# maltezfaria/LevelSetMethods.jl

Measured on AMD Instinct MI355X. Metric: Mcells/s per RK3 step (WENO5 advect+reinit), 512^3 fp64; HBM GB/s vs peak, higher is better.
Workload: dtype f64; 1 GPU; 3D 512^3 vortex-deformation WENO5 advection + EikonalReinitializationTerm, RK3, NeumannBC, fp64; cells=134217728, integrator=RK3, arithmetic_mode=fast, parallelism=single, halo_overlap=n/a, prewarm_steps=10, exchange=n/a

## Files before the change

### levelsetmethods.jl_amd/csrc/stage_kernel.h

```cpp
#pragma once
#include <cstdlib>
#include <type_traits>
#include "lsm_internal.h"
#include "stage_math.h"

namespace lsm {
namespace LSM_NS {

#if LSM_STRICT
#define LSM_LDS7 0
#define LSM_ZD 0
constexpr bool ADV_SCALED = false;
#else
constexpr bool ADV_SCALED = true;
#endif
constexpr int adv_factor_kind(int ADV, bool PLAIN) {
#if LSM_STRICT
    return 0;
#else
    return ADV == 2 ? (LSM_T1 ? 1 : 0) | (LSM_T2 && PLAIN ? 2 : 0) : 0;
#endif
}
template <int FK>
LSM_DEV double adv_factor(const StageArgs& a, int k) {
    if constexpr (FK == 3) return a.cdt_inv_h3[k];
    else if constexpr (FK == 2) return a.cdt * a.inv_h[k];
    else if constexpr (FK == 1) return a.inv_h3[k];
    else return a.inv_h[k];
}

constexpr int halo_of(int ADV, int NM, int CURV, int EIK) {
    int g = 0;
    if (ADV == 2) g = 3;
    if (ADV == 1 && g < 1) g = 1;
    if ((NM || EIK) && g < 2) g = 2;
    if (CURV && g < 1) g = 1;
    return g;
}

template <class T>
LSM_DEV T* uniform_ptr(T* p) {
    const unsigned long long v = reinterpret_cast<unsigned long long>(p);
    const unsigned lo = __builtin_amdgcn_readfirstlane((unsigned)v), hi = __builtin_amdgcn_readfirstlane((unsigned)(v >> 32));
    return reinterpret_cast<T*>(((unsigned long long)hi << 32) | lo);
}
LSM_DEV double ld_uniform(const double* t, int i) {
    typedef const __attribute__((address_space(4))) double* cptr;
    return *((cptr)(unsigned long long)t + i);
}
typedef unsigned lsm_v2u __attribute__((ext_vector_type(2)));
LSM_DEV __amdgpu_buffer_rsrc_t plane_rsrc(const void* base, int range = (int)0x80000000u) {
    return __builtin_amdgcn_make_buffer_rsrc(const_cast<void*>(base), 0, range, 0x00020000);
}
constexpr unsigned LSM_OOB_OFFSET = 0xC0000000u;
template <class ST, int AUX = 0>
LSM_DEV double ldg(const ST* base, unsigned boff, int range = (int)0x80000000u) {
    if constexpr (sizeof(ST) == 8) return __builtin_bit_cast(double, __builtin_amdgcn_raw_buffer_load_b64(plane_rsrc(base, range), boff, 0, AUX));
    else return (double)__builtin_bit_cast(float, __builtin_amdgcn_raw_buffer_load_b32(plane_rsrc(base, range), boff, 0, AUX));
}
template <class ST, int AUX = 0>
LSM_DEV void stg(ST* base, unsigned boff, double v) {
    if constexpr (sizeof(ST) == 8) __builtin_amdgcn_raw_buffer_store_b64(__builtin_bit_cast(lsm_v2u, v), plane_rsrc(base), boff, 0, AUX);
    else __builtin_amdgcn_raw_buffer_store_b32(__builtin_bit_cast(unsigned, (float)v), plane_rsrc(base), boff, 0, AUX);
}
typedef unsigned lsm_v4u __attribute__((ext_vector_type(4)));
template <class ST, int AUX = 0>
LSM_DEV void ldg2(const ST* base, unsigned boff, double& x, double& y, int range = (int)0x80000000u) {
    if constexpr (sizeof(ST) == 8) {
        const lsm_v4u v = __builtin_bit_cast(lsm_v4u, __builtin_amdgcn_raw_buffer_load_b128(plane_rsrc(base, range), boff, 0, AUX));
        x = __builtin_bit_cast(double, lsm_v2u{v.x, v.y});
        y = __builtin_bit_cast(double, lsm_v2u{v.z, v.w});
    } else {
        const unsigned long long u = __builtin_bit_cast(unsigned long long, __builtin_amdgcn_raw_buffer_load_b64(plane_rsrc(base, range), boff, 0, AUX));
        x = (double)__builtin_bit_cast(float, (unsigned)u);
        y = (double)__builtin_bit_cast(float, (unsigned)(u >> 32));
    }
}
template <class ST, int AUX = 0>
LSM_DEV void stg2(ST* base, unsigned boff, double x, double y) {
    if constexpr (sizeof(ST) == 8) {
        const lsm_v2u a = __builtin_bit_cast(lsm_v2u, x), b = __builtin_bit_cast(lsm_v2u, y);
        __builtin_amdgcn_raw_buffer_store_b128(lsm_v4u{a.x, a.y, b.x, b.y}, plane_rsrc(base), boff, 0, AUX);
    } else {
        const unsigned long long u = (unsigned long long)__builtin_bit_cast(unsigned, (float)x) | ((unsigned long long)__builtin_bit_cast(unsigned, (float)y) << 32);
        __builtin_amdgcn_raw_buffer_store_b64(__builtin_bit_cast(lsm_v2u, u), plane_rsrc(base), boff, 0, AUX);
    }
}
LSM_DEV unsigned ldg_u8(const unsigned char* base, unsigned boff, int range) {
    return __builtin_amdgcn_raw_buffer_load_b8(
        __builtin_amdgcn_make_buffer_rsrc(const_cast<unsigned char*>(base), 0, __builtin_amdgcn_readfirstlane(range), 0x00020000), boff, 0, 0);
}

template <int NDIM, int NCOMP, bool SCALED = false, int KIND = -1, int FK = 0>
LSM_DEV void coeff_prep(const CoeffArgs& c, const StageArgs& a, int gi0, int gi1, double pre[3]) {
    pre[0] = pre[1] = pre[2] = 0.0;
    const int kind = KIND >= 0 ? KIND : c.kind;
    if (kind == LSM_COEFF_CONST) {
#pragma unroll
        for (int k = 0; k < NCOMP; ++k) pre[k] = SCALED ? c.v[k] * adv_factor<FK>(a, k) : c.v[k];
    } else if (kind == LSM_COEFF_ROTATION) {
        const double x1 = a.lc[0] + (double)gi0 * a.h[0];
        pre[1] = c.v[0] * (x1 - c.v[1]);
        if (SCALED) pre[1] = pre[1] * adv_factor<FK>(a, 1);
        if (NDIM == 3) {
            const double x2 = a.lc[1] + (double)gi1 * a.h[1];
            pre[0] = -(c.v[0] * (x2 - c.v[2]));
            if (SCALED) pre[0] = pre[0] * adv_factor<FK>(a, 0);
        }
    } else if (kind == LSM_COEFF_SEPARABLE) {
#pragma unroll
        for (int k = 0; k < NCOMP; ++k) {
            const double* T = c.sep[k];
            double p = T[gi0];
            if (NDIM == 3) p = p * T[a.gn[0] + gi1];
            pre[k] = SCALED ? p * (c.tfac * adv_factor<FK>(a, k)) : p;
        }
    }
}
template <int NDIM, int NCOMP, bool SCALED = false, int KIND = -1, int FK = 0>
LSM_DEV void coeff_eval(const CoeffArgs& c, const StageArgs& a, const double pre[3], const double tz[3], int gim, long long plane_off,
                        unsigned ocol, double out[3]) {
    const int kind = KIND >= 0 ? KIND : c.kind;
    if (kind == LSM_COEFF_CONST) {
#pragma unroll
        for (int k = 0; k < NCOMP; ++k) out[k] = pre[k];
    } else if (kind == LSM_COEFF_ROTATION) {
        if (NDIM == 2) {
            const double x2 = a.lc[1] + (double)gim * a.h[1];
            out[0] = -(c.v[0] * (x2 - c.v[2]));
            if (SCALED) out[0] = out[0] * adv_factor<FK>(a, 0);
        } else {
            out[0] = pre[0];
        }
        if (NCOMP > 1) out[1] = pre[1];
        if (NCOMP > 2) out[2] = 0.0;
    } else if (kind == LSM_COEFF_SEPARABLE) {
#pragma unroll
        for (int k = 0; k < NCOMP; ++k) {
            double p = pre[k];
            if (NDIM > 1) p = p * tz[k];
            out[k] = SCALED ? p : p * c.tfac;
        }
    } else {
#pragma unroll
        for (int k = 0; k < NCOMP; ++k) {
            out[k] = ldg(uniform_ptr(c.f[k] + plane_off), ocol);
            if (SCALED) out[k] = out[k] * adv_factor<FK>(a, k);
        }
    }
}

struct PlaneTab {
    double adv[3], nm[3], curv[3];
};
template <int NDIM, int NCOMP, int KIND>
LSM_DEV void plane_tab_one(const CoeffArgs& c, const StageArgs& a, int gim, double tz[3]) {
    tz[0] = tz[1] = tz[2] = 1.0;
    if (NDIM > 1 && (KIND >= 0 ? KIND : c.kind) == LSM_COEFF_SEPARABLE) {
#pragma unroll
        for (int k = 0; k < NCOMP; ++k) tz[k] = ld_uniform(c.sep[k], (NDIM == 3 ? a.gn[0] + a.gn[1] : a.gn[0]) + gim);
    }
}
template <int NDIM, int ADV, int NM, int CURV, int AK>
LSM_DEV void plane_tab(const StageArgs& a, int gim, PlaneTab& t) {
    if constexpr (ADV != 0) plane_tab_one<NDIM, NDIM, AK>(a.adv, a, gim, t.adv);
    if constexpr (NM != 0) plane_tab_one<NDIM, 1, (AK >= 0 ? (int)LSM_COEFF_CONST : -1)>(a.nm, a, gim, t.nm);
    if constexpr (CURV != 0) plane_tab_one<NDIM, 1, (AK >= 0 ? (int)LSM_COEFF_CONST : -1)>(a.curv, a, gim, t.curv);
}

struct NodeIO {
    long long plane_off;
    unsigned ocol;
    unsigned ocold;
    int gim;
};

struct NodeOps {
    double u[3];
    double vnm;
    double bcurv;
    double s0;
    double phin;
    double out2;
    bool have_negs;
    unsigned long long negs[3];
};
template <int NDIM, int ADV, int NM, int CURV, int EIK, class ST, int AK>
LSM_DEV void node_operands(const StageArgs& a, const NodeIO& io, const double pre_adv[3], const double pre_nm[3],
                           const double pre_curv[3], const PlaneTab& pt, NodeOps& op) {
    op.u[0] = op.u[1] = op.u[2] = 0.0;
    op.vnm = op.bcurv = op.s0 = op.phin = op.out2 = 0.0;
    op.have_negs = false;
    if constexpr (ADV != 0)
        coeff_eval<NDIM, NDIM, ADV_SCALED, AK, adv_factor_kind(ADV, AK >= 0)>(a.adv, a, pre_adv, pt.adv, io.gim, io.plane_off, io.ocold, op.u);
    if constexpr (NM != 0) {
        double vv[3];
        coeff_eval<NDIM, 1, false, (AK >= 0 ? (int)LSM_COEFF_CONST : -1)>(a.nm, a, pre_nm, pt.nm, io.gim, io.plane_off, io.ocold, vv);
        op.vnm = vv[0];
    }
    if constexpr (CURV != 0) {
        double bb[3];
        coeff_eval<NDIM, 1, false, (AK >= 0 ? (int)LSM_COEFF_CONST : -1)>(a.curv, a, pre_curv, pt.curv, io.gim, io.plane_off, io.ocold, bb);
        op.bcurv = bb[0];
    }
    if constexpr (EIK == 1) op.s0 = ldg(uniform_ptr(a.s0 + io.plane_off), io.ocold);
    op.phin = ldg<ST, 0>(uniform_ptr(reinterpret_cast<const ST*>(a.phin) + io.plane_off), io.ocol,
                  __builtin_amdgcn_readfirstlane(a.base_mode == LSM_BASE_PSI ? 0 : (int)0x80000000u));
    if (AK < 0 && a.out2 && a.out2_accum) op.out2 = ldg(uniform_ptr(reinterpret_cast<const ST*>(a.out2) + io.plane_off), io.ocol);
}

template <int NDIM, int G, int W, int R = 0, int RN = 0, bool ZD_ = false>
struct NodeView {
    static constexpr bool ZD = ZD_;
    const double* T0;
    const double* Tm;
    const double* Tp;
    const double* zl;
    double c;
    LSM_DEV double z(int k) const {
        static_assert(!ZD_, "a ring of differences holds no march-axis values: dz()");
        return zl[RN > 0 ? (R + G + k + RN) % (RN > 0 ? RN : 1) : G + k];
    }
    LSM_DEV double dz(int k) const { return zl[(R + G + k + RN) % (RN > 0 ? RN : 1)]; }
    template <int D>
    LSM_DEV double at(int k) const {
        if constexpr (D == 0) return T0[k];
        else if constexpr (D == 1 && NDIM == 3) return T0[k * W];
        else {
            static_assert(!ZD_ || D < NDIM - 1, "a ring of differences holds no march-axis values");
            return z(k);
        }
    }
    template <int A, int B>
    LSM_DEV double corner(int sa, int sb) const {
        if constexpr (NDIM == 3 && A == 0 && B == 1) return T0[sa + sb * W];
        else {
            const double* P = sb > 0 ? Tp : Tm;
            if constexpr (A == 0) return P[sa];
            else return P[sa * W];
        }
    }
};

#if !LSM_STRICT
LSM_DEV double sel64(int m, double x, double y) {
    return __hiloint2double((__double2hiint(x) & m) | (__double2hiint(y) & ~m), (__double2loint(x) & m) | (__double2loint(y) & ~m));
}
#ifndef LSM_NO_UNIFORM_PATHS
#define LSM_UNIFORM_PATHS 1
#else
#define LSM_UNIFORM_PATHS 0
#endif
template <int NDIM, int D, int G, int W, bool PQ, class NV>
LSM_DEV double weno_term(const NV& nv, const StageArgs& a, double v, bool have_negs, unsigned long long negs_known, double& P, double& Q) {
    const double epsf = 1.0e-99 * a.h2[D];
    auto lds = [&](auto Sc) {
        constexpr int ss = (D == 0 ? 1 : W) * decltype(Sc)::value;
        const double q0 = nv.T0[-3 * ss], q1 = nv.T0[-2 * ss], q2 = nv.T0[-ss], q4 = nv.T0[ss], q5 = nv.T0[2 * ss];
        return weno5_undivided_pq<PQ, LSM_T1 != 0>(q1 - q0, q2 - q1, nv.c - q2, q4 - nv.c, q5 - q4, epsf, P, Q);
    };
    auto reg = [&](auto Sc) {
        constexpr int ss = decltype(Sc)::value;
        if constexpr (NV::ZD) {
            if constexpr (ss > 0)
                return weno5_undivided_pq<PQ, LSM_T1 != 0, true>(nv.dz(-3), nv.dz(-2), nv.dz(-1), nv.dz(0), nv.dz(1), epsf, P, Q,
                                                                 max_abs5(nv.dz(-3), nv.dz(-2), nv.dz(-1), nv.dz(0), nv.dz(1)));
            else
                return weno5_undivided_pq<PQ, LSM_T1 != 0, true>(-nv.dz(2), -nv.dz(1), -nv.dz(0), -nv.dz(-1), -nv.dz(-2), epsf, P, Q,
                                                                 max_abs5(nv.dz(2), nv.dz(1), nv.dz(0), nv.dz(-1), nv.dz(-2)));
        } else {
            return weno5_undivided_pq<PQ, LSM_T1 != 0>(nv.z(-2 * ss) - nv.z(-3 * ss), nv.z(-ss) - nv.z(-2 * ss), nv.c - nv.z(-ss),
                                          nv.z(ss) - nv.c, nv.z(2 * ss) - nv.z(ss), epsf, P, Q);
        }
    };
    constexpr bool IN_LDS = D == 0 || (D == 1 && NDIM == 3);
    double w;
    const unsigned long long negs = have_negs ? negs_known : __builtin_amdgcn_ballot_w64(__double2hiint(v) < 0);
    if (LSM_UNIFORM_PATHS && negs == 0) {
        if constexpr (IN_LDS) w = lds(std::integral_constant<int, 1>{});
        else w = reg(std::integral_constant<int, 1>{});
    } else if (LSM_UNIFORM_PATHS && negs == __builtin_amdgcn_ballot_w64(true)) {
        if constexpr (IN_LDS) w = lds(std::integral_constant<int, -1>{});
        else w = reg(std::integral_constant<int, -1>{});
    } else {
        const int m = ~(__double2hiint(v) >> 31);
        if constexpr (!IN_LDS && NV::ZD) {
            w = weno5_undivided_pq<PQ, LSM_T1 != 0>(sel64(m, nv.dz(-3), -nv.dz(2)), sel64(m, nv.dz(-2), -nv.dz(1)), sel64(m, nv.dz(-1), -nv.dz(0)),
                                                    sel64(m, nv.dz(0), -nv.dz(-1)), sel64(m, nv.dz(1), -nv.dz(-2)), epsf, P, Q);
        } else {
            double q[6];
            if constexpr (IN_LDS) {
                constexpr int st = D == 0 ? 1 : W;
                const int ss = (st & m) | (-st & ~m);
                q[0] = nv.T0[-3 * ss]; q[1] = nv.T0[-2 * ss]; q[2] = nv.T0[-ss];
                q[3] = nv.c;
                q[4] = nv.T0[ss]; q[5] = nv.T0[2 * ss];
            } else {
                q[0] = sel64(m, nv.z(-3), nv.z(3));
                q[1] = sel64(m, nv.z(-2), nv.z(2));
                q[2] = sel64(m, nv.z(-1), nv.z(1));
                q[3] = nv.c;
                q[4] = sel64(m, nv.z(1), nv.z(-1));
                q[5] = sel64(m, nv.z(2), nv.z(-2));
            }
            w = weno5_undivided_pq<PQ, LSM_T1 != 0>(q[1] - q[0], q[2] - q[1], q[3] - q[2], q[4] - q[3], q[5] - q[4], epsf, P, Q);
        }
    }
    return w;
}
#endif

template <int NDIM, int D, int G, int W, class NV>
LSM_DEV double weno_dim(const NV& nv, const StageArgs& a, double v) {
    const bool up = v > 0;
    double q[6];
    if constexpr (D == 0 || (D == 1 && NDIM == 3)) {
        constexpr int st = D == 0 ? 1 : W;
        const int ss = up ? st : -st;
        q[0] = nv.T0[-3 * ss]; q[1] = nv.T0[-2 * ss]; q[2] = nv.T0[-ss];
        q[3] = nv.c;
        q[4] = nv.T0[ss]; q[5] = nv.T0[2 * ss];
    } else {
        q[0] = up ? nv.z(-3) : nv.z(3);
        q[1] = up ? nv.z(-2) : nv.z(2);
        q[2] = up ? nv.z(-1) : nv.z(1);
        q[3] = nv.c;
        q[4] = up ? nv.z(1) : nv.z(-1);
        q[5] = up ? nv.z(2) : nv.z(-2);
    }
    const double hs = up ? a.h[D] : -a.h[D];
    const double ihs = up ? a.inv_h[D] : -a.inv_h[D];
    return weno5_upwind(q, hs, ihs, 1.0e-99 * a.h2[D]);
}

template <int NDIM, int ADV, int NM, int CURV, int EIK, int G, int W, class ST, bool PLAIN, class NV>
LSM_DEV void node_update(const StageArgs& a, const NV& nv, const NodeOps& op, double& r_out, double& r_out2) {
    const double c = nv.c;
    double Ladv = 0.0, Lnm = 0.0, Lcurv = 0.0, Leik = 0.0;
#if LSM_STRICT
    constexpr bool ADV_TO_BASE = false;
#else
    constexpr bool ADV_TO_BASE = (adv_factor_kind(ADV, PLAIN) & 2) != 0;
    constexpr bool EIK_RAW = LSM_T3 && EIK == 2;
#endif
    [[maybe_unused]] double adv_base = 0.0;
    double A[3] = {0, 0, 0}, B[3] = {0, 0, 0};
#if LSM_STRICT
    constexpr bool ENO_FROM_WENO = false;
#else
    constexpr bool ENO_FROM_WENO = ADV == 2 && (NM || EIK);
#endif

    if constexpr (ADV != 0) {
        const double* u = op.u;
        auto one = [&](auto Dc) {
            constexpr int D = decltype(Dc)::value;
            const double v = u[D];
            double der;
            if constexpr (ADV == 2) {
#if LSM_STRICT
                der = weno_dim<NDIM, D, G, W>(nv, a, v);
#else
                const double w = weno_term<NDIM, D, G, W, ENO_FROM_WENO>(nv, a, v, op.have_negs, op.negs[D], A[D], B[D]);
                if constexpr (ADV_TO_BASE) {
                    adv_base = D == 0 ? -(__builtin_fabs(v) * w) : __builtin_fma(-__builtin_fabs(v), w, adv_base);
                    return 0.0;
                } else {
                    return __builtin_fabs(v) * w;
                }
#endif
            } else {
#if LSM_STRICT
                der = v > 0 ? (c - nv.template at<D>(-1)) / a.h[D] : (nv.template at<D>(1) - c) / a.h[D];
#else
                der = v > 0 ? (c - nv.template at<D>(-1)) : (nv.template at<D>(1) - c);
#endif
            }
            return v * der;
        };
        Ladv = one(std::integral_constant<int, 0>{});
        if constexpr (NDIM > 1) Ladv = Ladv + one(std::integral_constant<int, 1>{});
        if constexpr (NDIM > 2) Ladv = Ladv + one(std::integral_constant<int, 2>{});
    }

    if constexpr ((NM || EIK) && !ENO_FROM_WENO) {
        auto pr = [&](auto Dc) {
            constexpr int D = decltype(Dc)::value;
            eno2_pair(nv.template at<D>(-2), nv.template at<D>(-1), c, nv.template at<D>(1), nv.template at<D>(2), a.h[D],
                      a.h2[D], a.inv_h[D], A[D], B[D]);
        };
        pr(std::integral_constant<int, 0>{});
        if constexpr (NDIM > 1) pr(std::integral_constant<int, 1>{});
        if constexpr (NDIM > 2) pr(std::integral_constant<int, 2>{});
    }

    if constexpr (NM) {
        const double v = op.vnm;
#if LSM_STRICT
        double gp = 0.0, gm = 0.0;
#pragma unroll
        for (int d = 0; d < NDIM; ++d) {
            double x = positive(A[d]) * positive(A[d]) + negative(B[d]) * negative(B[d]);
            double y = negative(A[d]) * negative(A[d]) + positive(B[d]) * positive(B[d]);
            if (d == 0) { gp = x; gm = y; } else { gp = gp + x; gm = gm + y; }
        }
        Lnm = positive(v) * lsm_sqrt(gp) + negative(v) * lsm_sqrt(gm);
#else
        double g2 = 0.0;
        const unsigned long long vpos = __builtin_amdgcn_ballot_w64(v > 0);
        if (LSM_UNIFORM_PATHS && vpos == __builtin_amdgcn_ballot_w64(true)) {
            g2 = godunov_sum<NDIM, true>(A, B, a.inv_h2, a.uniform_h != 0);
        } else if (LSM_UNIFORM_PATHS && vpos == 0) {
            g2 = godunov_sum<NDIM, false>(A, B, a.inv_h2, a.uniform_h != 0);
        } else {
            const double sg = v > 0 ? 1.0 : -1.0;
#pragma unroll
            for (int d = 0; d < NDIM; ++d) g2 += godunov_term(sg, A[d], B[d], a.inv_h2[d]);
        }
        Lnm = v * fast_norm(g2);
#endif
    }

    if constexpr (CURV) {
        const double bb[1] = {op.bcurv};
#if LSM_STRICT
        double gr[3] = {0, 0, 0}, Hd[3] = {0, 0, 0};
        double H01 = 0, H02 = 0, H12 = 0;
        auto first = [&](auto Dc) {
            constexpr int D = decltype(Dc)::value;
            const double p1 = nv.template at<D>(1), m1 = nv.template at<D>(-1);
            gr[D] = (p1 - m1) / (2 * a.h[D]);
            Hd[D] = (p1 - 2 * c + m1) / a.h2[D];
        };
        first(std::integral_constant<int, 0>{});
        if constexpr (NDIM > 1) first(std::integral_constant<int, 1>{});
        if constexpr (NDIM > 2) first(std::integral_constant<int, 2>{});
        auto mixed = [&](auto Ac, auto Bc) {
            constexpr int A_ = decltype(Ac)::value, B_ = decltype(Bc)::value;
            const double pp = nv.template corner<A_, B_>(1, 1), pm = nv.template corner<A_, B_>(1, -1);
            const double mp = nv.template corner<A_, B_>(-1, 1), mm = nv.template corner<A_, B_>(-1, -1);
            return ((pp - pm) / (2 * a.h[B_]) - (mp - mm) / (2 * a.h[B_])) / (2 * a.h[A_]);
// ... 184 lines not shown
__device__ __forceinline__ void stage_tile(const StageArgs& a, unsigned tile_id, bool tail_tile, unsigned slot) {
    constexpr bool PLAIN = AK >= 0;
    constexpr bool NOMASK = PLAIN && !MASKED;
    constexpr int CK = PLAIN ? (int)LSM_COEFF_CONST : -1;
    constexpr int G = halo_of(ADV, NM, CURV, EIK);
    constexpr bool HAS_Y = NDIM == 3, MARCH = NDIM >= 2;
    constexpr int LEAD = (CURV && MARCH) ? 1 : 0;
    constexpr bool ZROT = LSM_ZROT && !LSM_STRICT && NDIM == 3 && ADV == 2;
    constexpr int W = TX + 2 * G;
    constexpr int H = HAS_Y ? TY + 2 * G : 1;
    constexpr int HW = H * W;
    constexpr bool LDS7 = LSM_LDS7 && ZROT && LEAD == 0 && PLAIN && !MASKED && !NM && EIK == 2 && (2 * G + 1) * HW * 8 + 64 <= 32768;
    constexpr bool ZD = LSM_ZD && LDS7;
    constexpr int NSLOT = LDS7 ? 2 * G + 1 : (MARCH ? 2 * LEAD + 2 : 1);
    constexpr int NT = TX * TY;
    constexpr int NHX = 2 * G * TY;
    constexpr int WY = CURV ? W : TX;
    constexpr int NHY = HAS_Y ? 2 * G * WY : 0;
    constexpr int NH = NHX + NHY;
    constexpr int HPT = (NH + NT - 1) / NT;
    static_assert(!HAS_Y || TY > 1 || true, "");
    __shared__ double tile[NSLOT * HW];

#ifdef LSM_STAMP
    const unsigned long long st_rb = __builtin_amdgcn_s_memrealtime();
#endif
    if (a.tile_list) tile_id = (unsigned)a.tile_list[tile_id];
    else if (a.tile_active && !a.tile_active[tile_id]) return;
    const unsigned tbx = tile_id % a.nb[0], tby = (tile_id / a.nb[0]) % a.nb[1];
    const unsigned tbm = tile_id / (a.nb[0] * a.nb[1]);

    const int tid = threadIdx.x;
    int tx = tid % TX, ty = tid / TX;
    if constexpr (NDIM == 3 && TX == 32 && TY == 8 && !NOMASK) {
        if (LSM_BAND_PATCH && a.mask) { tx = 8 * (tid >> 6) + (tid & 7); ty = (tid & 63) >> 3; }
    }
    const int bx0 = tbx * TX, by0 = HAS_Y ? tby * TY : 0;
    const int gx = bx0 + tx, gy = by0 + ty;
    const int nx = a.n[0], ny = HAS_Y ? a.n[1] : 1;
    const int nm = MARCH ? a.n[NDIM - 1] : 1;
    const long long sy = HAS_Y ? a.s1 : 0;
    const long long sm = MARCH ? (NDIM == 3 ? a.s2 : a.s1) : 0;
    const bool active = gx < nx && gy < ny;
    const int cx = gx < nx ? gx : nx - 1, cy = gy < ny ? gy : ny - 1;
    const int xk0 = a.xkind[0], xk1 = a.xkind[1], yk0 = a.ykind[0], yk1 = a.ykind[1];
    const bool xmap = a.xredirect && (bx0 < G || bx0 + TX + G > nx);
    const bool ymap = HAS_Y && a.yredirect && (by0 < G || by0 + TY + G > ny);
    auto bsrc = [](int i, int n, int k0, int k1) {
        const bool left = i < 0;
        const int k = left ? -i : i - (n - 1), kind = left ? k0 : k1;
        const int per = left ? (n - 1) - k : k, ext = left ? 0 : n - 1, sym = left ? k : (n - 1) - k;
        return kind == LSM_BC_PERIODIC ? per : (kind == LSM_BC_EXTRAPOLATION ? ext : sym);
    };
    auto xsrc = [&](int i) { return (!xmap || (i >= 0 && i < nx)) ? i : bsrc(i, nx, xk0, xk1); };
    auto ysrc = [&](int i) { return (!ymap || (i >= 0 && i < ny)) ? i : bsrc(i, ny, yk0, yk1); };
    const int lxg = xsrc(gx < nx + G ? gx : nx + G - 1);
    const int lyg = HAS_Y ? ysrc(gy < ny + G ? gy : ny + G - 1) : 0;
    const long long corner = a.origin - G - (HAS_Y ? (long long)G * sy : 0);
    const unsigned ocole = (unsigned)(lxg + G) + (unsigned)(lyg + (HAS_Y ? G : 0)) * (unsigned)sy;
    const unsigned ocol = (unsigned)sizeof(ST) * ocole, ocold = 8u * ocole;
    const int mcl = a.mc > 0 ? a.mc : MC;
    const int mc = tail_tile ? a.mc_tail : mcl;
    const int m0 = MARCH ? (tail_tile ? a.mb + (int)a.nbig * mcl + (int)(tbm - a.nbig) * mc : a.mb + (int)tbm * mc) : 0;
    const int m1 = MARCH ? (m0 + mc < a.me ? m0 + mc : a.me) : 1;
    const int mlo = (MARCH && a.mredirect[0]) ? 0 : -G, mhi = (MARCH && a.mredirect[1]) ? nm - 1 : nm + G - 1;
    auto clampM = [&](int p) { return p < mlo ? mlo : (p > mhi ? mhi : p); };
    auto plane = [&](int p) { return uniform_ptr(reinterpret_cast<const ST*>(a.psi) + (corner + (long long)clampM(p) * sm)); };

    int hl[HPT > 0 ? HPT : 1];
    unsigned hg[HPT > 0 ? HPT : 1];
    bool hv[HPT > 0 ? HPT : 1];
#pragma unroll
    for (int h = 0; h < HPT; ++h) {
        const int e = tid + h * NT;
        hv[h] = e < NH;
        int lx, ly;
        if (e < NHX) {
            const int r = e % (2 * G);
            ly = e / (2 * G) + (HAS_Y ? G : 0);
            lx = r < G ? r : r + TX;
        } else {
            const int e2 = e - NHX;
            const int row = e2 / WY;
            lx = (CURV ? 0 : G) + e2 % WY;
            ly = row < G ? row : row + TY;
        }
        int X = bx0 - G + lx;
        X = xsrc(X > nx + G - 1 ? nx + G - 1 : X);
        int Y = 0;
        if (HAS_Y) {
            Y = by0 - G + ly;
            Y = ysrc(Y > ny + G - 1 ? ny + G - 1 : Y);
        }
        hl[h] = ly * W + lx;
        hg[h] = (unsigned)sizeof(ST) * ((unsigned)(X + G) + (unsigned)(Y + (HAS_Y ? G : 0)) * (unsigned)sy);
        if (!hv[h]) hg[h] = LSM_OOB_OFFSET;
    }
    const int lpos = (ty + (HAS_Y ? G : 0)) * W + tx + G;

    double pre_adv[3] = {0, 0, 0}, pre_nm[3] = {0, 0, 0}, pre_curv[3] = {0, 0, 0};
    {
        const int gi0 = cx + a.goff[0], gi1 = HAS_Y ? cy + a.goff[1] : 0;
        if constexpr (ADV != 0) coeff_prep<NDIM, NDIM, ADV_SCALED, AK, adv_factor_kind(ADV, PLAIN)>(a.adv, a, gi0, gi1, pre_adv);
        if constexpr (NM != 0) coeff_prep<NDIM, 1, false, CK>(a.nm, a, gi0, gi1, pre_nm);
        if constexpr (CURV != 0) coeff_prep<NDIM, 1, false, CK>(a.curv, a, gi0, gi1, pre_curv);
    }

    if constexpr (!MARCH) {
        const ST* P = plane(0);
        const double c = ldg(P, ocol);
        const NodeIO io{corner, ocol, ocold, 0};
        NodeOps op;
        PlaneTab pt;
        plane_tab<NDIM, ADV, NM, CURV, AK>(a, 0, pt);
        node_operands<NDIM, ADV, NM, CURV, EIK, ST, AK>(a, io, pre_adv, pre_nm, pre_curv, pt, op);
        tile[lpos] = c;
#pragma unroll
        for (int h = 0; h < HPT; ++h)
            if (hv[h]) tile[hl[h]] = ldg(P, hg[h]);
        __syncthreads();
        NodeView<NDIM, G, W> nv{tile + lpos, nullptr, nullptr, nullptr, c};
        double r1, r2;
        node_update<NDIM, ADV, NM, CURV, EIK, G, W, ST, PLAIN>(a, nv, op, r1, r2);
        node_store<ST, PLAIN>(a, io, active && (NOMASK || !a.mask || ldg_u8(uniform_ptr(a.mask + corner), ocold >> 3, (int)0x80000000u) != 0), r1, r2);
    } else {
        PlaneTab pt;
        plane_tab<NDIM, ADV, NM, CURV, AK>(a, m0 + a.goff[NDIM - 1], pt);
        double zl[2 * G + 1];
#pragma unroll
        for (int j = 0; j <= 2 * G; ++j) zl[j] = ldg(plane(m0 - G + j), ocol);
        double hp[2 * LEAD + 1][HPT > 0 ? HPT : 1];
#pragma unroll
        for (int pl = -LEAD; pl <= LEAD; ++pl) {
            const ST* P = plane(m0 + pl);
#pragma unroll
            for (int h = 0; h < HPT; ++h) hp[pl + LEAD][h] = ldg(P, hg[h]);
        }
#pragma unroll
        for (int pl = -LEAD; pl <= LEAD; ++pl) {
            const int slot = pl + LEAD;
            tile[slot * HW + lpos] = zl[G + pl];
#pragma unroll
            for (int h = 0; h < HPT; ++h)
                if (hv[h]) tile[slot * HW + hl[h]] = hp[slot][h];
        }
        [[maybe_unused]] double zlast = 0.0;
        if constexpr (ZD) {
#pragma unroll
            for (int s = 1; s <= G; ++s) tile[s * HW + lpos] = zl[G + s];
            zlast = zl[2 * G];
#pragma unroll
            for (int j = 0; j < 2 * G; ++j) zl[j] = zl[j + 1] - zl[j];
        }
        const bool nomask = NOMASK || a.mask == nullptr;
        const int mrange = nomask ? 0 : (int)0x80000000u;
        long long po = corner + (long long)m0 * sm;
        unsigned mk_next = 0;
        if constexpr (!NOMASK) mk_next = ldg_u8(uniform_ptr(a.mask + po), ocold >> 3, mrange);
        const ST* Pnx = plane(m0 + G);
        const ST* Pn = plane(m0 + LEAD);
        const int plast = mhi;
        const bool any_active = __builtin_amdgcn_ballot_w64(active) != 0;
        constexpr bool SIGNS_KNOWN = PLAIN && ADV == 2 && AK != LSM_COEFF_FIELD && !LSM_STRICT;
        unsigned long long neg_pre[3] = {0, 0, 0};
        const unsigned long long all_lanes = __builtin_amdgcn_ballot_w64(true);
        if constexpr (SIGNS_KNOWN) {
#pragma unroll
            for (int d = 0; d < NDIM; ++d) neg_pre[d] = __builtin_amdgcn_ballot_w64(__double2hiint(pre_adv[d]) < 0);
        }
        __builtin_amdgcn_s_waitcnt(0x0F70);
#ifdef LSM_STAMP
        const unsigned long long st_t0 = __builtin_amdgcn_s_memtime(), st_r0 = __builtin_amdgcn_s_memrealtime();
#endif
        constexpr int ROT = ZROT ? 2 * G + 1 : 0, RM = ROT > 0 ? ROT : 1;
        auto plane_iter = [&](auto Rc, int m) {
            constexpr int R = decltype(Rc)::value;
            Pnx = uniform_ptr(m + 1 + G <= plast ? Pnx + sm : Pnx);
            Pn = uniform_ptr(m + 1 + LEAD <= plast ? Pn + sm : Pn);
            const double nxt = ldg(Pnx, ocol);
            double hn[HPT > 0 ? HPT : 1];
#pragma unroll
            for (int h = 0; h < HPT; ++h) hn[h] = ldg(Pn, hg[h]);
            const unsigned mk = mk_next;
            if constexpr (!NOMASK) mk_next = ldg_u8(uniform_ptr(a.mask + (po + sm)), ocold >> 3, mrange);
            const NodeIO io{po, ocol, ocold, m + a.goff[NDIM - 1]};
            NodeOps op;
            node_operands<NDIM, ADV, NM, CURV, EIK, ST, AK>(a, io, pre_adv, pre_nm, pre_curv, pt, op);
            if constexpr (SIGNS_KNOWN) {
                op.have_negs = true;
#pragma unroll
                for (int d = 0; d < NDIM; ++d) {
                    if (AK == LSM_COEFF_SEPARABLE) op.negs[d] = neg_pre[d] ^ (__double2hiint(pt.adv[d]) < 0 ? all_lanes : 0ull);
                    else op.negs[d] = neg_pre[d];
                }
                if (AK == LSM_COEFF_ROTATION) op.have_negs = NDIM == 3;
            }
            LSM_BARRIER();
            const bool on = active && (nomask || mk != 0);
            double r1 = 0.0, r2 = 0.0;
            if (NOMASK ? any_active : __builtin_amdgcn_ballot_w64(on) != 0) {
                const int rel = m - m0;
                const double* T0 = tile + (LDS7 ? R : (rel + LEAD) % NSLOT) * HW + lpos;
                const double* Tm = tile + ((rel + LEAD + NSLOT - 1) % NSLOT) * HW + lpos;
                const double* Tp = tile + ((rel + LEAD + 1) % NSLOT) * HW + lpos;
                NodeView<NDIM, G, W, R, ROT, ZD> nv{T0, LDS7 ? nullptr : Tm, LDS7 ? nullptr : Tp, zl, ZD ? T0[0] : zl[ROT > 0 ? (R + G) % RM : G]};
                node_update<NDIM, ADV, NM, CURV, EIK, G, W, ST, PLAIN>(a, nv, op, r1, r2);
            }
            plane_tab<NDIM, ADV, NM, CURV, AK>(a, (m + 1 < m1 ? m + 1 : m) + a.goff[NDIM - 1], pt);
            if constexpr (ZD) {
                zl[(R + 2 * G) % RM] = nxt - zlast;
                zlast = nxt;
            } else if constexpr (ROT > 0) {
                zl[R % RM] = nxt;
            } else {
#pragma unroll
                for (int j = 0; j < 2 * G; ++j) zl[j] = zl[j + 1];
                zl[2 * G] = nxt;
            }
            const int wslot = LDS7 ? (R + 1) % NSLOT : (m - m0 + 1 + 2 * LEAD) % NSLOT;
            if constexpr (ZD) tile[((R + G + 1) % NSLOT) * HW + lpos] = nxt;
            else tile[wslot * HW + lpos] = zl[ROT > 0 ? (R + 1 + G + LEAD) % RM : G + LEAD];
#pragma unroll
            for (int h = 0; h < HPT; ++h)
                if (hv[h]) tile[wslot * HW + hl[h]] = hn[h];
            node_store<ST, PLAIN>(a, io, on, r1, r2);
            po += sm;
        };
        if constexpr (ROT > 0) {
            int m = m0;
            while (m < m1) {
                bool go = true;
                auto step = [&](auto Rc) {
                    if (go) {
                        plane_iter(Rc, m);
                        ++m;
                        go = m < m1;
                    }
                };
                step(std::integral_constant<int, 0>{});
                step(std::integral_constant<int, 1>{});
                step(std::integral_constant<int, 2>{});
                if constexpr (ROT > 3) step(std::integral_constant<int, 3>{});
                if constexpr (ROT > 4) step(std::integral_constant<int, 4>{});
                if constexpr (ROT > 5) step(std::integral_constant<int, 5>{});
                if constexpr (ROT > 6) step(std::integral_constant<int, 6>{});
                if constexpr (ROT > 7) step(std::integral_constant<int, 7>{});
            }
        } else {
            for (int m = m0; m < m1; ++m) plane_iter(std::integral_constant<int, 0>{}, m);
        }
#ifdef LSM_STAMP
        if (a.stamp && threadIdx.x == 0) {
            const unsigned long long st_t1 = __builtin_amdgcn_s_memtime(), st_r1 = __builtin_amdgcn_s_memrealtime();
            a.stamp[4 * (slot % 16384u)] = st_t1 - st_t0;
            a.stamp[4 * (slot % 16384u) + 1] = st_rb;
            a.stamp[4 * (slot % 16384u) + 2] = st_r0;
            a.stamp[4 * (slot % 16384u) + 3] = st_r1;
        }
#endif
    }
}

struct TileOrder {
    unsigned ntiles, nbigt, big_per, small_per;
    __host__ __device__ explicit TileOrder(const StageArgs& a) {
        ntiles = a.tile_list ? a.ntile_list : a.nb[0] * a.nb[1] * a.nb[2];
        nbigt = a.mc_tail > 0 ? a.nb[0] * a.nb[1] * a.nbig : ntiles;
        big_per = (nbigt + 7u) / 8u;
        small_per = (ntiles - nbigt + 7u) / 8u;
    }
    __host__ __device__ unsigned per_xcd() const { return big_per + small_per; }
    __host__ __device__ bool entry(unsigned x, unsigned j, unsigned& id, bool& tail) const {
        const unsigned nb = x * big_per < nbigt ? (nbigt - x * big_per < big_per ? nbigt - x * big_per : big_per) : 0u;
        if (j < nb) { id = x * big_per + j; tail = false; return true; }
        const unsigned js = j - nb, so = nbigt + x * small_per;
        if (so + js < ntiles && js < small_per) { id = so + js; tail = true; return true; }
        return false;
    }
};

template <int NDIM, int ADV, int NM, int CURV, int EIK, int TX, int TY, int MC, class ST, int AK, bool MASKED>
__global__ void __launch_bounds__(TX* TY, (LSM_ZROT && !LSM_STRICT && NDIM == 3 && ADV == 2 && AK >= 0 && !MASKED && !CURV && !NM) ? 5 : LSM_WAVES_PER_EU)
    stage_kernel(const StageArgs a) {
    const TileOrder ord(a);
    unsigned tile_id;
    bool tail_tile;
    if (NDIM == 3 && !MASKED && a.tail_wgs && blockIdx.x >= 8u * ord.big_per) {
        __shared__ unsigned s_ticket;
        if (threadIdx.x == 0) {
            const unsigned t = __hip_atomic_fetch_add(a.tail_ctr, 1u, __ATOMIC_RELAXED, __HIP_MEMORY_SCOPE_AGENT);
            if (t + 1u == a.tail_wgs) __hip_atomic_store(a.tail_ctr, 0u, __ATOMIC_RELAXED, __HIP_MEMORY_SCOPE_AGENT);
            s_ticket = t;
        }
        __syncthreads();
        const unsigned t = (unsigned)__builtin_amdgcn_readfirstlane((int)s_ticket);
        if (t >= ord.ntiles - ord.nbigt) return;
        tile_id = ord.nbigt + t;
        tail_tile = true;
    } else if (!ord.entry(blockIdx.x % 8u, blockIdx.x / 8u, tile_id, tail_tile)) {
        return;
    }
    stage_tile<NDIM, ADV, NM, CURV, EIK, TX, TY, MC, ST, AK, MASKED>(a, tile_id, tail_tile, blockIdx.x);
}

template <int ADV, int NM, int CURV, int EIK, int TX, int TY, int MC, class ST>
__device__ __forceinline__ void stage_tile2(const StageArgs& a, unsigned tile_id) {
    constexpr int NDIM = 3;
    constexpr int AK = LSM_COEFF_CONST;
    static_assert(!CURV, "stage_tile2 serves the axis-aligned single terms; curvature stays with stage_tile (see the comment above)");
    constexpr int G = halo_of(ADV, NM, CURV, EIK);
    constexpr int NSLOT = 2;
    constexpr int TXN = 2 * TX;
    constexpr int W = TXN + 2 * G, H = TY + 2 * G, HW = H * W, NT = TX * TY;
    constexpr int NHX = 2 * G * TY;
    constexpr int WY = TXN;
    constexpr int NHY = 2 * G * WY;
    constexpr int NH = NHX + NHY;
    constexpr int HPT = (NH + NT - 1) / NT;
    __shared__ double tile[NSLOT * HW];

    const unsigned tbx = tile_id % a.nb[0], tby = (tile_id / a.nb[0]) % a.nb[1], tbm = tile_id / (a.nb[0] * a.nb[1]);
    const int tid = threadIdx.x, tx = tid % TX, ty = tid / TX;
    const int bx0 = tbx * TXN, by0 = tby * TY;
    const int gx = bx0 + 2 * tx, gy = by0 + ty;
    const int nx = a.n[0], ny = a.n[1], nm = a.n[2];
    const long long sy = a.s1, sm = a.s2;
    const bool active = gx < nx && gy < ny;
    const int xk0 = a.xkind[0], xk1 = a.xkind[1], yk0 = a.ykind[0], yk1 = a.ykind[1];
    const bool xmap = a.xredirect && (bx0 < G || bx0 + TXN + G > nx);
    const bool ymap = a.yredirect && (by0 < G || by0 + TY + G > ny);
    auto bsrc = [](int i, int n, int k0, int k1) {
        const bool left = i < 0;
        const int k = left ? -i : i - (n - 1), kind = left ? k0 : k1;
        const int per = left ? (n - 1) - k : k, ext = left ? 0 : n - 1, sym = left ? k : (n - 1) - k;
        return kind == LSM_BC_PERIODIC ? per : (kind == LSM_BC_EXTRAPOLATION ? ext : sym);
    };
    auto xsrc = [&](int i) { return (!xmap || (i >= 0 && i < nx)) ? i : bsrc(i, nx, xk0, xk1); };
    auto ysrc = [&](int i) { return (!ymap || (i >= 0 && i < ny)) ? i : bsrc(i, ny, yk0, yk1); };
    const bool whole = bx0 + TXN <= nx;
    const int lyg = ysrc(gy < ny + G ? gy : ny + G - 1);
    const int lx0 = xsrc(gx < nx + G ? gx : nx + G - 1), lx1 = xsrc(gx + 1 < nx + G ? gx + 1 : nx + G - 1);
    const long long corner = a.origin - G - (long long)G * sy;
    const unsigned orow = (unsigned)(lyg + G) * (unsigned)sy;
    const unsigned ocole0 = (unsigned)(lx0 + G) + orow, ocole1 = (unsigned)(lx1 + G) + orow;
    const unsigned ocol0 = (unsigned)sizeof(ST) * ocole0, ocol1 = (unsigned)sizeof(ST) * ocole1, ocold0 = 8u * ocole0;
    const int mc = a.mc > 0 ? a.mc : MC;
    const int m0 = a.mb + (int)tbm * mc;
    const int m1 = m0 + mc < a.me ? m0 + mc : a.me;
    const int mlo = a.mredirect[0] ? 0 : -G, mhi = a.mredirect[1] ? nm - 1 : nm + G - 1;
    auto clampM = [&](int p) { return p < mlo ? mlo : (p > mhi ? mhi : p); };
    auto plane = [&](int p) { return uniform_ptr(reinterpret_cast<const ST*>(a.psi) + (corner + (long long)clampM(p) * sm)); };
    auto ldpair = [&](const ST* P, double& x, double& y) {
        if (whole) ldg2(P, ocol0, x, y);
        else { x = ldg(P, ocol0); y = ldg(P, ocol1); }
    };

    int hl[HPT];
    unsigned hg[HPT];
    bool hv[HPT];
#pragma unroll
// ... 275 lines not shown
```

### levelsetmethods.jl_amd/csrc/stage_math.h

```cpp
#pragma once
#include <hip/hip_runtime.h>

namespace lsm {
namespace LSM_NS {

#define LSM_DEV __device__ __forceinline__

LSM_DEV double positive(double x) { return x > 0.0 ? x : 0.0; }
LSM_DEV double negative(double x) { return x < 0.0 ? x : 0.0; }

#if LSM_STRICT

LSM_DEV double jl_max(double a, double b) { return (a != a || b != b) ? __builtin_nan("") : (b > a ? b : a); }

LSM_DEV double weno5_core(double v1, double v2, double v3, double v4, double v5) {
    double dphi1 = (1.0 / 3) * v1 - (7.0 / 6) * v2 + (11.0 / 6) * v3;
    double dphi2 = -(1.0 / 6) * v2 + (5.0 / 6) * v3 + (1.0 / 3) * v4;
    double dphi3 = (1.0 / 3) * v3 + (5.0 / 6) * v4 - (1.0 / 6) * v5;
    double a1 = v1 - 2 * v2 + v3, b1 = v1 - 4 * v2 + 3 * v3;
    double a2 = v2 - 2 * v3 + v4, b2 = v2 - v4;
    double a3 = v3 - 2 * v4 + v5, b3 = 3 * v3 - 4 * v4 + v5;
    double S1 = (13.0 / 12) * (a1 * a1) + (1.0 / 4) * (b1 * b1);
    double S2 = (13.0 / 12) * (a2 * a2) + (1.0 / 4) * (b2 * b2);
    double S3 = (13.0 / 12) * (a3 * a3) + (1.0 / 4) * (b3 * b3);
    double m = jl_max(jl_max(jl_max(jl_max(v1 * v1, v2 * v2), v3 * v3), v4 * v4), v5 * v5);
    double eps = 1.0e-6 * m + 1.0e-99;
    double t1 = S1 + eps, t2 = S2 + eps, t3 = S3 + eps;
    double al1 = 0.1 / (t1 * t1);
    double al2 = 0.6 / (t2 * t2);
    double al3 = 0.3 / (t3 * t3);
    double w1 = al1 / (al1 + al2 + al3);
    double w2 = al2 / (al1 + al2 + al3);
    double w3 = al3 / (al1 + al2 + al3);
    return w1 * dphi1 + w2 * dphi2 + w3 * dphi3;
}

LSM_DEV double limiter(double x, double y) {
    if (!(x * y > 0.0)) return 0.0;
    return __builtin_fabs(x) <= __builtin_fabs(y) ? x : y;
}

LSM_DEV double weno5_upwind(const double q[6], double hs, double , double ) {
    return weno5_core((q[1] - q[0]) / hs, (q[2] - q[1]) / hs, (q[3] - q[2]) / hs, (q[4] - q[3]) / hs,
                      (q[5] - q[4]) / hs);
}

LSM_DEV void eno2_pair(double m2, double m1, double c, double p1, double p2, double h, double h2, double ,
                       double& A, double& B) {
    double dm = (c - m1) / h;
    double dp = (p1 - c) / h;
    double d20 = (p1 - 2 * c + m1) / h2;
    double d2mm = (m2 - 2 * m1 + c) / h2;
    double d2pp = (c - 2 * p1 + p2) / h2;
    A = dm + 0.5 * h * limiter(d2mm, d20);
    B = dp - 0.5 * h * limiter(d2pp, d20);
}
LSM_DEV double lsm_sqrt(double x) { return __builtin_sqrt(x); }
LSM_DEV double lsm_div(double a, double b) { return a / b; }

#else

#ifndef LSM_T1
#define LSM_T1 1
#endif
#ifndef LSM_T2
#define LSM_T2 1
#endif
#ifndef LSM_T3
#define LSM_T3 1
#endif
#ifndef LSM_LDS7
#define LSM_LDS7 1
#endif
#ifndef LSM_ZD
#define LSM_ZD 1
#endif

LSM_DEV double fast_rcp(double x) {
    double r = __builtin_amdgcn_rcp(x);
    double e = __builtin_fma(-x, r, 1.0);
    return __builtin_fma(r, e, r);
}
LSM_DEV double lsm_div(double a, double b) { return a * fast_rcp(b); }

LSM_DEV double fast_rsqrt(double x) {
    double r = __builtin_amdgcn_rsq(x);
    double e = __builtin_fma(-0.5 * x * r, r, 0.5);
    return __builtin_fma(r, e, r);
}

LSM_DEV double fast_norm(double x) { return x * fast_rsqrt(__builtin_fmax(x, 1.0e-300)); }

LSM_DEV double lsm_sqrt(double x0) {
    const double x = __builtin_fmax(x0, 1.0e-300);
    double r = __builtin_amdgcn_rsq(x);
    double g = x * r, hh = 0.5 * r;
    double e = __builtin_fma(-hh, g, 0.5);
    g = __builtin_fma(g, e, g);
    hh = __builtin_fma(hh, e, hh);
    double d = __builtin_fma(-g, g, x);
    return __builtin_fma(d, hh, g);
}

LSM_DEV double minmod_fast(double x, double y);
LSM_DEV double max_abs5(double e1, double e2, double e3, double e4, double e5) {
    double a, b, m;
    asm("v_max_f64 %0, |%1|, |%2|" : "=v"(a) : "v"(e1), "v"(e2));
    asm("v_max_f64 %0, |%1|, |%2|" : "=v"(b) : "v"(e3), "v"(e4));
    asm("v_max_f64 %0, %1, %2" : "=v"(m) : "v"(a), "v"(b));
    asm("v_max_f64 %0, %1, |%2|" : "=v"(m) : "v"(m), "v"(e5));
    return m;
}
template <bool PQ, bool X3 = false, bool MPRE = false>
LSM_DEV double weno5_undivided_pq(double e1, double e2, double e3, double e4, double e5, double eps_floor, double& P, double& Q, double m_pre = 0.0) {
    const double w1 = e2 - e1, w2 = e3 - e2, w3 = e4 - e3, w4 = e5 - e4;
    if constexpr (PQ) {
        const double hi = __builtin_fmax(w3, 0.0), lo = __builtin_fmin(w3, 0.0);
        P = __builtin_fma(0.5, __builtin_fmax(__builtin_fmin(w2, hi), lo), e3);
        Q = __builtin_fma(-0.5, __builtin_fmax(__builtin_fmin(w4, hi), lo), e4);
    }
    const double A1 = w2 - w1, A2 = w3 - w2, A3 = w4 - w3;
    const double m = MPRE ? m_pre
                          : __builtin_fmax(__builtin_fmax(__builtin_fmax(__builtin_fabs(e1), __builtin_fabs(e2)),
                                                          __builtin_fmax(__builtin_fabs(e3), __builtin_fabs(e4))),
                                           __builtin_fabs(e5));
    const double eps = __builtin_fma(0.75e-6 * m, m, (13.0 / 16) * __builtin_fmax(eps_floor, 1.0e-75));
    const double t2 = 0.75 * w2, t3 = 0.75 * w3;
    const double r1 = __builtin_fma(A1, A1, __builtin_fma(t2, A1 + w2, eps));
    const double r2 = __builtin_fma(A2, A2, __builtin_fma(t2, w3, eps));
    const double r3 = __builtin_fma(A3, A3, __builtin_fma(t3, w3 - A3, eps));
    const double s1 = r1 * r1, s2 = r2 * r2, s3 = r3 * r3;
    const double N = s2 * __builtin_fma(1.5, s1 * (A2 - A3), s3 * (A1 - A2));
    const double Dn = __builtin_fma(6.0, s1 * s3, s2 * __builtin_fma(3.0, s1, s3));
    if constexpr (X3) return __builtin_fma(fast_rcp(Dn), N, __builtin_fma(0.5, w2, __builtin_fma(3.0, e3, w3)));
    const double dphi2 = __builtin_fma(1.0 / 3, w3, __builtin_fma(1.0 / 6, w2, e3));
    return __builtin_fma(fast_rcp(Dn) * (1.0 / 3), N, dphi2);
}
LSM_DEV double weno5_undivided(double e1, double e2, double e3, double e4, double e5, double eps_floor) {
    double P, Q;
    return weno5_undivided_pq<false>(e1, e2, e3, e4, e5, eps_floor, P, Q);
}

LSM_DEV double weno5_upwind(const double q[6], double , double inv_hs, double eps_floor) {
    return weno5_undivided(q[1] - q[0], q[2] - q[1], q[3] - q[2], q[4] - q[3], q[5] - q[4], eps_floor) * inv_hs;
}

LSM_DEV double minmod_fast(double x, double y) {
    return __builtin_fmax(__builtin_fmin(x, y), __builtin_fmin(__builtin_fmax(x, y), 0.0));
}

LSM_DEV void eno2_pair(double m2, double m1, double c, double p1, double p2, double , double , double ,
                       double& A, double& B) {
    const double dm = c - m1, dp = p1 - c;
    const double s0 = dp - dm;
    const double smm = dm - (m1 - m2);
    const double spp = (p2 - p1) - dp;
    const double hi = __builtin_fmax(s0, 0.0), lo = __builtin_fmin(s0, 0.0);
    A = __builtin_fma(0.5, __builtin_fmax(__builtin_fmin(smm, hi), lo), dm);
    B = __builtin_fma(-0.5, __builtin_fmax(__builtin_fmin(spp, hi), lo), dp);
}
#endif

#if LSM_STRICT
LSM_DEV void godunov_sel(bool vpos, double A, double B, double& a2, double& b2) {
    double a = vpos ? positive(A) : negative(A);
    double b = vpos ? negative(B) : positive(B);
    a2 = a * a;
    b2 = b * b;
}
#else
LSM_DEV double godunov_term(double sg, double A, double B, double inv_h2) {
    const double a = __builtin_fmax(sg * A, 0.0);
    const double b = __builtin_fmin(sg * B, 0.0);
    return __builtin_fma(a, a, b * b) * inv_h2;
}
LSM_DEV double vmax0(double x) { double r; asm("v_max_f64 %0, %1, 0" : "=v"(r) : "v"(x)); return r; }
LSM_DEV double vmin0(double x) { double r; asm("v_min_f64 %0, %1, 0" : "=v"(r) : "v"(x)); return r; }
LSM_DEV double godunov_pos(double A, double B, double inv_h2) {
    const double a = vmax0(A);
    const double b = vmin0(B);
    return __builtin_fma(a, a, b * b) * inv_h2;
}
LSM_DEV double godunov_neg(double A, double B, double inv_h2) {
    const double a = vmin0(A);
    const double b = vmax0(B);
    return __builtin_fma(a, a, b * b) * inv_h2;
}
template <int NDIM, bool POS, bool RAW = false>
LSM_DEV double godunov_sum(const double* A, const double* B, const double* inv_h2, bool uniform_h) {
    if (RAW || uniform_h) {
        double s = 0.0;
#pragma unroll
        for (int d = 0; d < NDIM; ++d) {
            const double a = POS ? vmax0(A[d]) : vmin0(A[d]);
            const double b = POS ? vmin0(B[d]) : vmax0(B[d]);
            s = d == 0 ? a * a : __builtin_fma(a, a, s);
            s = __builtin_fma(b, b, s);
        }
        if constexpr (RAW) return s;
        return s * inv_h2[0];
    }
    double s = 0.0;
#pragma unroll
    for (int d = 0; d < NDIM; ++d) s += POS ? godunov_pos(A[d], B[d], inv_h2[d]) : godunov_neg(A[d], B[d], inv_h2[d]);
    return s;
}
LSM_DEV double vmax_floor(double x) { double r; asm("v_max_f64 %0, %1, %2" : "=v"(r) : "v"(x), "s"(1.0e-300)); return r; }
LSM_DEV double godunov_term_raw(double sg, double A, double B) {
    const double a = __builtin_fmax(sg * A, 0.0);
    const double b = __builtin_fmin(sg * B, 0.0);
    return __builtin_fma(a, a, b * b);
}
LSM_DEV void eikonal_tail_raw(double sf, double c, double& root, double& S) {
    const double r = __builtin_amdgcn_rsq(sf);
    const double g = sf * r, hh = 0.5 * r;
    const double q = __builtin_fma(-g, hh, 0.5);
    root = __builtin_fma(g, q, g);
    S = c * fast_rsqrt(__builtin_fma(c, c, sf));
}
#endif

}
}
```

Baseline: 42730 Mcells/s.

## Carry march-axis minmod across planes, unify WENO eps floor, precompute LDS slot bases

Three default-on micro-optimizations are added to the WENO5 stage kernel. EPS1 computes a single epsilon floor from the maximum grid spacing for all axes, which saves per-axis loads but slightly changes the numerics. ZA computes the minmod limiter for the march (z) axis only once per plane and carries it in a register to the next plane, roughly halving the limiter work for that axis. SLOTBASE precomputes 32-bit LDS addresses for each tile slot so address arithmetic is not redone in the march loop, at the cost of more registers.

```diff
diff --git a/levelsetmethods.jl_amd/csrc/stage_kernel.h b/levelsetmethods.jl_amd/csrc/stage_kernel.h
--- a/levelsetmethods.jl_amd/csrc/stage_kernel.h
+++ b/levelsetmethods.jl_amd/csrc/stage_kernel.h
@@ -10,6 +10,9 @@
 #if LSM_STRICT
 #define LSM_LDS7 0
 #define LSM_ZD 0
+#define LSM_EPS1 0
+#define LSM_ZA 0
+#define LSM_SLOTBASE 0
 constexpr bool ADV_SCALED = false;
 #else
 constexpr bool ADV_SCALED = true;
@@ -217,6 +220,8 @@
     const double* Tp;
     const double* zl;
     double c;
+    double zmc = 0.0;
+    double* zmn = nullptr;
     LSM_DEV double z(int k) const {
         static_assert(!ZD_, "a ring of differences holds no march-axis values: dz()");
         return zl[RN > 0 ? (R + G + k + RN) % (RN > 0 ? RN : 1) : G + k];
@@ -253,7 +258,9 @@
 #endif
 template <int NDIM, int D, int G, int W, bool PQ, class NV>
 LSM_DEV double weno_term(const NV& nv, const StageArgs& a, double v, bool have_negs, unsigned long long negs_known, double& P, double& Q) {
-    const double epsf = 1.0e-99 * a.h2[D];
+    constexpr bool EPS1 = LSM_EPS1 && NV::ZD && NDIM == 3;
+    const double epsf = 1.0e-99 * (EPS1 ? __builtin_fmax(__builtin_fmax(a.h2[0], a.h2[1]), a.h2[NDIM - 1]) : a.h2[D]);
+    [[maybe_unused]] constexpr bool ZA = LSM_ZA && NV::ZD && PQ && D == NDIM - 1;
     auto lds = [&](auto Sc) {
         constexpr int ss = (D == 0 ? 1 : W) * decltype(Sc)::value;
         const double q0 = nv.T0[-3 * ss], q1 = nv.T0[-2 * ss], q2 = nv.T0[-ss], q4 = nv.T0[ss], q5 = nv.T0[2 * ss];
@@ -263,11 +270,11 @@
         constexpr int ss = decltype(Sc)::value;
         if constexpr (NV::ZD) {
             if constexpr (ss > 0)
-                return weno5_undivided_pq<PQ, LSM_T1 != 0, true>(nv.dz(-3), nv.dz(-2), nv.dz(-1), nv.dz(0), nv.dz(1), epsf, P, Q,
-                                                                 max_abs5(nv.dz(-3), nv.dz(-2), nv.dz(-1), nv.dz(0), nv.dz(1)));
+                return weno5_undivided_pq<PQ, LSM_T1 != 0, true, ZA ? 1 : 0>(nv.dz(-3), nv.dz(-2), nv.dz(-1), nv.dz(0), nv.dz(1), epsf, P, Q,
+                                                                 max_abs5(nv.dz(-3), nv.dz(-2), nv.dz(-1), nv.dz(0), nv.dz(1)), nv.zmc, nv.zmn);
             else
-                return weno5_undivided_pq<PQ, LSM_T1 != 0, true>(-nv.dz(2), -nv.dz(1), -nv.dz(0), -nv.dz(-1), -nv.dz(-2), epsf, P, Q,
-                                                                 max_abs5(nv.dz(2), nv.dz(1), nv.dz(0), nv.dz(-1), nv.dz(-2)));
+                return weno5_undivided_pq<PQ, LSM_T1 != 0, true, ZA ? -1 : 0>(-nv.dz(2), -nv.dz(1), -nv.dz(0), -nv.dz(-1), -nv.dz(-2), epsf, P, Q,
+                                                                 max_abs5(nv.dz(2), nv.dz(1), nv.dz(0), nv.dz(-1), nv.dz(-2)), nv.zmc, nv.zmn);
         } else {
             return weno5_undivided_pq<PQ, LSM_T1 != 0>(nv.z(-2 * ss) - nv.z(-3 * ss), nv.z(-ss) - nv.z(-2 * ss), nv.c - nv.z(-ss),
                                           nv.z(ss) - nv.c, nv.z(2 * ss) - nv.z(ss), epsf, P, Q);
@@ -285,8 +292,8 @@
     } else {
         const int m = ~(__double2hiint(v) >> 31);
         if constexpr (!IN_LDS && NV::ZD) {
-            w = weno5_undivided_pq<PQ, LSM_T1 != 0>(sel64(m, nv.dz(-3), -nv.dz(2)), sel64(m, nv.dz(-2), -nv.dz(1)), sel64(m, nv.dz(-1), -nv.dz(0)),
-                                                    sel64(m, nv.dz(0), -nv.dz(-1)), sel64(m, nv.dz(1), -nv.dz(-2)), epsf, P, Q);
+            w = weno5_undivided_pq<PQ, LSM_T1 != 0, false, ZA ? 2 : 0>(sel64(m, nv.dz(-3), -nv.dz(2)), sel64(m, nv.dz(-2), -nv.dz(1)), sel64(m, nv.dz(-1), -nv.dz(0)),
+                                                    sel64(m, nv.dz(0), -nv.dz(-1)), sel64(m, nv.dz(1), -nv.dz(-2)), epsf, P, Q, 0.0, nv.zmc, nv.zmn, m, nv.dz(-1), nv.dz(0), nv.dz(1));
         } else {
             double q[6];
             if constexpr (IN_LDS) {
@@ -777,6 +784,21 @@
 #pragma unroll
             for (int j = 0; j < 2 * G; ++j) zl[j] = zl[j + 1] - zl[j];
         }
+        [[maybe_unused]] double zcar = 0.0;
+        if constexpr (ZD && LSM_ZA) {
+            const double w2 = zl[G - 1] - zl[G - 2], w3 = zl[G] - zl[G - 1];
+            zcar = __builtin_fmax(__builtin_fmin(w2, __builtin_fmax(w3, 0.0)), __builtin_fmin(w3, 0.0));
+        }
+        constexpr bool SLOTBASE = LSM_SLOTBASE && ZD && AK == LSM_COEFF_SEPARABLE && 6 * W <= 255;
+        typedef const __attribute__((address_space(3))) double* lds_cptr;
+        [[maybe_unused]] unsigned sbase[NSLOT];
+        if constexpr (SLOTBASE) {
+#pragma unroll
+            for (int k = 1; k < NSLOT; ++k) {
+                sbase[k] = (unsigned)(unsigned long long)(lds_cptr)(tile + k * HW + lpos - G * W);
+                asm volatile("" : "+v"(sbase[k]));
+            }
+        }
         const bool nomask = NOMASK || a.mask == nullptr;
         const int mrange = nomask ? 0 : (int)0x80000000u;
         long long po = corner + (long long)m0 * sm;
@@ -823,14 +845,17 @@
             LSM_BARRIER();
             const bool on = active && (nomask || mk != 0);
             double r1 = 0.0, r2 = 0.0;
+            [[maybe_unused]] double zmm = __builtin_nondeterministic_value(zcar);
             if (NOMASK ? any_active : __builtin_amdgcn_ballot_w64(on) != 0) {
                 const int rel = m - m0;
                 const double* T0 = tile + (LDS7 ? R : (rel + LEAD) % NSLOT) * HW + lpos;
+                if constexpr (SLOTBASE && R > 0) T0 = (const double*)(lds_cptr)(unsigned long long)sbase[R % NSLOT] + G * W;
                 const double* Tm = tile + ((rel + LEAD + NSLOT - 1) % NSLOT) * HW + lpos;
                 const double* Tp = tile + ((rel + LEAD + 1) % NSLOT) * HW + lpos;
-                NodeView<NDIM, G, W, R, ROT, ZD> nv{T0, LDS7 ? nullptr : Tm, LDS7 ? nullptr : Tp, zl, ZD ? T0[0] : zl[ROT > 0 ? (R + G) % RM : G]};
+                NodeView<NDIM, G, W, R, ROT, ZD> nv{T0, LDS7 ? nullptr : Tm, LDS7 ? nullptr : Tp, zl, ZD ? T0[0] : zl[ROT > 0 ? (R + G) % RM : G], zcar, &zmm};
                 node_update<NDIM, ADV, NM, CURV, EIK, G, W, ST, PLAIN>(a, nv, op, r1, r2);
             }
+            if constexpr (ZD && LSM_ZA) zcar = zmm;
             plane_tab<NDIM, ADV, NM, CURV, AK>(a, (m + 1 < m1 ? m + 1 : m) + a.goff[NDIM - 1], pt);
             if constexpr (ZD) {
                 zl[(R + 2 * G) % RM] = nxt - zlast;
diff --git a/levelsetmethods.jl_amd/csrc/stage_math.h b/levelsetmethods.jl_amd/csrc/stage_math.h
--- a/levelsetmethods.jl_amd/csrc/stage_math.h
+++ b/levelsetmethods.jl_amd/csrc/stage_math.h
@@ -75,6 +75,15 @@
 #ifndef LSM_ZD
 #define LSM_ZD 1
 #endif
+#ifndef LSM_EPS1
+#define LSM_EPS1 1
+#endif
+#ifndef LSM_ZA
+#define LSM_ZA 1
+#endif
+#ifndef LSM_SLOTBASE
+#define LSM_SLOTBASE 1
+#endif
 
 LSM_DEV double fast_rcp(double x) {
     double r = __builtin_amdgcn_rcp(x);
@@ -111,10 +120,27 @@
     asm("v_max_f64 %0, %1, |%2|" : "=v"(m) : "v"(m), "v"(e5));
     return m;
 }
-template <bool PQ, bool X3 = false, bool MPRE = false>
-LSM_DEV double weno5_undivided_pq(double e1, double e2, double e3, double e4, double e5, double eps_floor, double& P, double& Q, double m_pre = 0.0) {
+template <bool PQ, bool X3 = false, bool MPRE = false, int CAR = 0>
+LSM_DEV double weno5_undivided_pq(double e1, double e2, double e3, double e4, double e5, double eps_floor, double& P, double& Q, double m_pre = 0.0,
+                                  double mc = 0.0, double* mnext = nullptr, int lm = 0, double im = 0.0, double i0 = 0.0, double i1 = 0.0) {
     const double w1 = e2 - e1, w2 = e3 - e2, w3 = e4 - e3, w4 = e5 - e4;
-    if constexpr (PQ) {
+    if constexpr (PQ && CAR != 0) {
+        const double hi = __builtin_fmax(w3, 0.0), lo = __builtin_fmin(w3, 0.0);
+        const double mm = __builtin_fmax(__builtin_fmin(CAR == 2 ? i1 - i0 : (CAR > 0 ? w4 : w2), hi), lo);
+        *mnext = mm;
+        if constexpr (CAR == 1) {
+            P = __builtin_fma(0.5, mc, e3);
+            Q = __builtin_fma(-0.5, mm, e4);
+        } else if constexpr (CAR == -1) {
+            P = __builtin_fma(0.5, mm, e3);
+            Q = __builtin_fma(-0.5, mc, e4);
+        } else {
+            const double dm = __builtin_fma(0.5, mc, im), dp = __builtin_fma(-0.5, mm, i0);
+            const int sb = (int)0x80000000u;
+            P = __hiloint2double((__double2hiint(dm) & lm) | ((__double2hiint(dp) ^ sb) & ~lm), (__double2loint(dm) & lm) | (__double2loint(dp) & ~lm));
+            Q = __hiloint2double((__double2hiint(dp) & lm) | ((__double2hiint(dm) ^ sb) & ~lm), (__double2loint(dp) & lm) | (__double2loint(dm) & ~lm));
+        }
+    } else if constexpr (PQ) {
         const double hi = __builtin_fmax(w3, 0.0), lo = __builtin_fmin(w3, 0.0);
         P = __builtin_fma(0.5, __builtin_fmax(__builtin_fmin(w2, hi), lo), e3);
         Q = __builtin_fma(-0.5, __builtin_fmax(__builtin_fmin(w4, hi), lo), e4);
```

Result: no change. 43000 Mcells/s (median of 6 runs) (+0.6%).
